# Sindhu-Hegde/jegal

Hardware: AMD Instinct MI355X
Metric: clips/sec (T=150 frames, 270x480) embedding extraction (higher is better)
Workload: dtype f16; 1 GPU; BASELINE configs[1]: synthetic batch=32 gesture-only (GestSync conv + JEGAL gesture encoder), uint8 150x270x480x3 clips resident in HBM, seeded synthetic weights; clips_per_gpu=32, frames=150, precision_mode=5, chunk=32, conv1_zero_tile_skip=True, dual_stream=True, parallelism=clip-sharded x1, no data-path collective

## Files before the change

### jegal_amd/csrc/conv1.hip

```cpp
#include "common.h"

#ifdef JG_CLOCK_STAMPS
__device__ unsigned long long jg_clock_stamps_conv1[2 * 1024];
extern "C" int jg_clock_read_conv1(unsigned long long* out, int n) {
    return hipMemcpyFromSymbol(out, HIP_SYMBOL(jg_clock_stamps_conv1), sizeof(unsigned long long) * (n < 2048 ? n : 2048)) == hipSuccess ? 0 : 1;
}
#endif
#include <cstdio>
#include <cstdlib>
#include <cstring>

struct Conv1Args {
    const uint8_t* src;
    int nclip, T, pad, P;
    const f16* Wd;
    float scale;
    f16* out;
    f16* edge;
    f16* dump;
    int nstrips;
    float invP;
    int zskip;
    const unsigned* zmask;
    const f16* zconst;
    int fill_partial;
};

namespace {
constexpr int IH = 270, IW = 480;
constexpr int PH = 43, PW = 78;
constexpr int TROWS = 16;
constexpr int ROW_PITCH = 3744;
constexpr int TILE_BYTES = TROWS * ROW_PITCH;
__device__ __host__ constexpr int slot_off(int x) { return 32 * x + 16 * (x / 3); }
constexpr int ROW_TILES = 22, COL_TILES = 5;
constexpr int CONV_BYTES = 4 * 8 * 32 * 16;
constexpr int CARRY_BYTES = 8 * 32 * 16;
constexpr int OFF_CONV = 2 * TILE_BYTES;
constexpr int OFF_CARRY = OFF_CONV + 2 * CONV_BYTES;
constexpr int OFF_INIT = OFF_CARRY + 2 * CARRY_BYTES;
constexpr int OFF_LIVE = OFF_INIT + 32;
constexpr int OFF_SKIP = OFF_INIT + 256;
constexpr int MAX_WG_STRIPS = 640;
constexpr int LDS_BYTES = OFF_SKIP + 4 * MAX_WG_STRIPS;
constexpr int MAX_WGS = 1024;
constexpr int DUMP_HALVES_PER_WG = 256 * 8;
}

typedef uint32_t u32x3 __attribute__((ext_vector_type(3)));
struct C1Regs { u32x3 w[2][5]; };

__device__ __forceinline__ f16x8 max8(f16x8 a, f16x8 b) {
    return __builtin_elementwise_max(a, b);
}

__device__ __forceinline__ int conv1_s2_of_mask(unsigned sk) {
    const int L = __builtin_ctz(~sk);
    constexpr int C2_OH = (PH - 5) / 2 + 1;
    const int rs = L >= 2 ? L - 2 : 0;
    return rs < C2_OH ? rs : C2_OH - 1;
}

struct Strips {
    int s_lo, r_hi, GX;
    const unsigned* tab;
    bool use_skip;
    __device__ __forceinline__ bool any() const { return s_lo < r_hi && GX > 0; }
    __device__ __forceinline__ unsigned zero_bands(int k) const {
        return use_skip ? (unsigned)__builtin_amdgcn_readfirstlane((int)tab[k]) : 0u;
    }
};
__device__ __forceinline__ Strips conv1_strips(const Conv1Args& a, const char* smem) {
    const int G32 = (int)gridDim.x;
    const int xcd = blockIdx.x & 7, xidx = blockIdx.x >> 3;
    const int GX = (G32 + 7 - xcd) >> 3;
    const int per = (a.nstrips + 7) >> 3;
    const int r_lo = xcd * per, r_hi = (r_lo + per < a.nstrips) ? r_lo + per : a.nstrips;
    return Strips{r_lo + xidx, r_hi, GX, reinterpret_cast<const unsigned*>(smem + OFF_SKIP), a.zmask != nullptr};
}
__device__ __forceinline__ void strip_split(int strip, int& nf, int& j) {
    nf = (int)((unsigned)strip / 5u);
    j = strip - nf * 5;
}
__device__ __forceinline__ unsigned skip_of(unsigned z) { return z & ((z << 1) | 1u); }
struct Walk {
    int strip, rt;
    int k;
    unsigned skip;
    unsigned z;
    bool done;
};
template <class F>
__device__ __forceinline__ void walk_next(const Strips& S, Walk& q, F&& on_strip) {
    if (q.done) return;
    while (true) {
        if (++q.rt == ROW_TILES) {
            q.rt = 0;
            q.strip += S.GX;
            ++q.k;
            if (q.strip >= S.r_hi) { q.done = true; return; }
            q.z = S.zero_bands(q.k);
            q.skip = skip_of(q.z);
            on_strip(q.strip, q.skip);
        }
        if (!((q.skip >> q.rt) & 1u)) return;
    }
}
template <class F>
__device__ __forceinline__ Walk walk_first(const Strips& S, F&& on_strip) {
    Walk q = {S.s_lo, -1, 0, 0u, 0u, !S.any()};
    if (q.done) return q;
    q.z = S.zero_bands(0);
    q.skip = skip_of(q.z);
    on_strip(q.strip, q.skip);
    walk_next(S, q, on_strip);
    return q;
}

__device__ __forceinline__ bool tile_live(const char* smem, int t) {
    return __builtin_amdgcn_readfirstlane(*reinterpret_cast<const int*>(smem + OFF_LIVE + (t & 1) * 4)) != 0;
}
__device__ __forceinline__ bool tile_is_zero(const char* smem, int t) {
    const int4 fl = *reinterpret_cast<const int4*>(smem + OFF_INIT + (t & 1) * 16);
    return __builtin_amdgcn_readfirstlane(fl.x | fl.y | fl.z | fl.w) == 0;
}

struct Mfma32 {
    static constexpr int NSTEP = 49, NCB = 1;
    static constexpr int DEPTH = 6;
    typedef f32x16 Acc;
    const int chalf, r, h;
    f16x8 wreg[49];
    const char* base;
    __device__ __forceinline__ Mfma32(const f16* Wd, int lane, int chalf_) : chalf(chalf_), r(lane & 31), h(lane >> 5) {
#pragma unroll
        for (int s = 0; s < 49; ++s)
            wreg[s] = *reinterpret_cast<const f16x8*>(Wd + conv1_wd_index(s, chalf * 32 + r, 8 * h));
    }
    __device__ __forceinline__ void set_tile(const char* cur) { base = cur + 112 * r + 16 * h; }
    __device__ __forceinline__ f16x8 frag(int gi) const {
        const int q = gi / 49, s = gi - q * 49;
        const int kh = s / 7, kw = s - kh * 7;
        return *reinterpret_cast<const f16x8*>(base + (6 * q + kh) * ROW_PITCH + 32 * kw + 16 * (kw / 3));
    }
    __device__ __forceinline__ static void zero(Acc& acc) {
#pragma unroll
        for (int x = 0; x < 16; ++x) acc[x] = 0.f;
    }
    __device__ __forceinline__ void step(Acc& acc, int s, int, f16x8 f) const {
        acc = __builtin_amdgcn_mfma_f32_32x32x16_f16(wreg[s], f, acc, 0, 0, 0);
    }
    __device__ __forceinline__ void store(const Acc& acc, char* cbuf, int mb, float scale) const {
#pragma unroll
        for (int g = 0; g < 4; ++g) {
            const f16x4 hv = {(f16)fmaxf(acc[4 * g] * scale, 0.f), (f16)fmaxf(acc[4 * g + 1] * scale, 0.f),
                              (f16)fmaxf(acc[4 * g + 2] * scale, 0.f), (f16)fmaxf(acc[4 * g + 3] * scale, 0.f)};
            *reinterpret_cast<f16x4*>(cbuf + ((mb * 8 + chalf * 4 + g) * 32 + r) * 16 + 8 * h) = hv;
        }
    }
};
struct Mfma16 {
    static constexpr int NSTEP = 25, NCB = 2;
    static constexpr int DEPTH = 4;
    struct Acc { f32x4 v[2][2]; };
    const int chalf, n16, kq, sel, half, colp;
    f16x8 wreg[25][2];
    int lb_row, lb_32, lb_224;
    int st_off;
    const char *p_row, *p_32, *p_224;
    __device__ __forceinline__ static void step_slots(int t, int& kha, int& kwa, int& khb, int& kwb) {
        if (t < 21) { kha = 2 * (t / 7); kwa = t % 7; khb = kha + 1; kwb = kwa; }
        else if (t == 21) { kha = khb = 6; kwa = 1; kwb = 2; }
        else if (t == 22) { kha = khb = 6; kwa = 4; kwb = 5; }
        else if (t == 23) { kha = khb = 6; kwa = 0; kwb = 6; }
        else { kha = khb = 6; kwa = 3; kwb = 4; }
    }
    __device__ __forceinline__ Mfma16(const f16* Wd, int lane, int chalf_)
        : chalf(chalf_), n16(lane & 15), kq(lane >> 4), sel(kq & 1), half(kq >> 1),
          colp((n16 >= 4 && n16 < 12) ? 2 * (n16 - 4) : (n16 < 4 ? 2 * n16 + 1 : 2 * (n16 - 8) + 1)) {
#pragma unroll
        for (int t = 0; t < 25; ++t) {
            int kha, kwa, khb, kwb;
            step_slots(t, kha, kwa, khb, kwb);
            const int sl = sel ? khb * 7 + kwb : kha * 7 + kwa;
#pragma unroll
            for (int ob = 0; ob < 2; ++ob) {
                wreg[t][ob] = *reinterpret_cast<const f16x8*>(Wd + conv1_wd_index(sl, chalf * 32 + ob * 16 + n16, 8 * half));
                if (t == 24 && sel) wreg[t][ob] = f16x8{0, 0, 0, 0, 0, 0, 0, 0};
            }
        }
        const int lb = 112 * colp + 16 * half;
        lb_row = lb + sel * ROW_PITCH; lb_32 = lb + sel * 32; lb_224 = lb + sel * 224;
        st_off = ((chalf * 4 + (kq >> 1)) * 32 + colp) * 16 + 8 * (kq & 1);
    }
    __device__ __forceinline__ void set_tile(const char* cur) {
        p_row = cur + lb_row;
        p_32 = cur + lb_32;
        p_224 = cur + lb_224;
    }
    __device__ __forceinline__ f16x8 frag(int gi) const {
        const int q = gi / 50, st = (gi - q * 50) >> 1, cb = gi & 1;
        int kha, kwa, khb, kwb;
        step_slots(st, kha, kwa, khb, kwb);
        const int off = (6 * q + kha) * ROW_PITCH + 32 * kwa + 16 * (kwa / 3) + 1792 * cb;
        const char* pb = st < 21 ? p_row : (st == 23 ? p_224 : p_32);
        return *reinterpret_cast<const f16x8*>(pb + off);
    }
    __device__ __forceinline__ static void zero(Acc& acc) {
#pragma unroll
        for (int ob = 0; ob < 2; ++ob)
#pragma unroll
            for (int cb = 0; cb < 2; ++cb) acc.v[ob][cb] = f32x4{0.f, 0.f, 0.f, 0.f};
    }
    __device__ __forceinline__ void step(Acc& acc, int st, int cb, f16x8 f) const {
        acc.v[0][cb] = __builtin_amdgcn_mfma_f32_16x16x32_f16(wreg[st][0], f, acc.v[0][cb], 0, 0, 0);
        acc.v[1][cb] = __builtin_amdgcn_mfma_f32_16x16x32_f16(wreg[st][1], f, acc.v[1][cb], 0, 0, 0);
    }
    __device__ __forceinline__ void store(const Acc& acc, char* cbuf, int mb, float scale) const {
#pragma unroll
        for (int ob = 0; ob < 2; ++ob)
#pragma unroll
            for (int cb = 0; cb < 2; ++cb) {
                const f32x4 v = acc.v[ob][cb];
                const f16x4 hv = {(f16)fmaxf(v.x * scale, 0.f), (f16)fmaxf(v.y * scale, 0.f), (f16)fmaxf(v.z * scale, 0.f), (f16)fmaxf(v.w * scale, 0.f)};
                *reinterpret_cast<f16x4*>(cbuf + st_off + ((mb * 8 + ob * 2) * 32 + cb * 16) * 16) = hv;
            }
    }
};

template <class Form>
__device__ __forceinline__ void conv1_mfma_role(const f16* Wd, float scale, char* smem, int lane, int wave) {
    constexpr int NSTEP = Form::NSTEP, NCB = Form::NCB, DEPTH = Form::DEPTH, NFRAG = 2 * NSTEP * NCB;
    const int mb0 = (wave >> 1) & 1;
    Form F(Wd, lane, wave & 1);
#ifdef JG_CLOCK_STAMPS
    const unsigned long long ck0 = __builtin_amdgcn_s_memtime(), rt0 = __builtin_amdgcn_s_memrealtime();
#endif
    for (int t = 0;; ++t) {
        __syncthreads();
        if (!tile_live(smem, t)) break;
        F.set_tile(smem + (t & 1) * TILE_BYTES + 3 * mb0 * ROW_PITCH);
        char* cbuf = smem + OFF_CONV + (t & 1) * CONV_BYTES;
        if (tile_is_zero(smem, t)) {
#pragma unroll
            for (int q = 0; q < 2; ++q) {
                typename Form::Acc acc;
                Form::zero(acc);
#pragma unroll
                for (int st = 0; st < 2; ++st)
#pragma unroll
                    for (int cb = 0; cb < NCB; ++cb) F.step(acc, st, cb, F.frag((q * NSTEP + st) * NCB + cb));
                F.store(acc, cbuf, mb0 + 2 * q, scale);
            }
            continue;
        }
        f16x8 fr[DEPTH];
#pragma unroll
        for (int gi = 0; gi < DEPTH; ++gi) fr[gi] = F.frag(gi);
#pragma unroll
        for (int q = 0; q < 2; ++q) {
            typename Form::Acc acc;
            Form::zero(acc);
#pragma unroll
            for (int st = 0; st < NSTEP; ++st)
#pragma unroll
                for (int cb = 0; cb < NCB; ++cb) {
                    const int gi = (q * NSTEP + st) * NCB + cb;
                    F.step(acc, st, cb, fr[gi % DEPTH]);
                    if (gi + DEPTH < NFRAG) fr[gi % DEPTH] = F.frag(gi + DEPTH);
                    __builtin_amdgcn_sched_barrier(0);
                }
            F.store(acc, cbuf, mb0 + 2 * q, scale);
        }
    }
#ifdef JG_CLOCK_STAMPS
    if (wave == 0 && lane == 0 && blockIdx.x < 1024) {
        jg_clock_stamps_conv1[2 * blockIdx.x] = __builtin_amdgcn_s_memtime() - ck0;
        jg_clock_stamps_conv1[2 * blockIdx.x + 1] = __builtin_amdgcn_s_memrealtime() - rt0;
    }
#endif
}

template <bool M16>
__global__ __launch_bounds__(512, 2) void conv1_direct_kernel(Conv1Args a) {
    extern __shared__ __attribute__((aligned(16))) char smem[];
    const int tid = threadIdx.x, lane = tid & 63;
    const int wave = __builtin_amdgcn_readfirstlane(tid >> 6);
    const Strips S = conv1_strips(a, smem);
    if (!S.any()) return;
    if (S.use_skip) {
        unsigned* tab = reinterpret_cast<unsigned*>(smem + OFF_SKIP);
        for (int k = tid; k < MAX_WG_STRIPS; k += 512) {
            const int strip = S.s_lo + k * S.GX;
            int nf, j;
            strip_split(strip, nf, j);
            tab[k] = strip < S.r_hi ? a.zmask[nf] : 0u;
        }
        __syncthreads();
    }
    if (wave >= 4) {
        const int ltid = tid - 256;
        const int row0 = ltid / 25, g0 = ltid - row0 * 25;
        const int it1 = ltid + 256;
        const bool has1 = it1 < TROWS * 25;
        const int row1 = has1 ? it1 / 25 : 0, g1 = has1 ? it1 - row1 * 25 : 0;

        uint32_t fb0_lo = (uint32_t)(uintptr_t)a.src, fb0_hi = (uint32_t)((uintptr_t)a.src >> 32);
        uint32_t fdelta[5] = {0, 0, 0, 0, 0};
        uint32_t ioff[2] = {0, 0};
        auto decode = [&](int strip, int& nf, int& j, int& b, int& pp) {
            strip_split(strip, nf, j);
            b = (int)((float)nf * a.invP);
            pp = nf - b * a.P;
            if (pp < 0) { --b; pp += a.P; }
            else if (pp >= a.P) { ++b; pp -= a.P; }
        };
        auto strip_setup = [&](int strip) {
            int nf, j, b, p;
            decode(strip, nf, j, b, p);
            int f0 = p - a.pad;
            f0 = f0 < 0 ? 0 : (f0 > a.T - 1 ? a.T - 1 : f0);
            const uintptr_t fb = (uintptr_t)(a.src + (size_t)(b * a.T + f0) * (size_t)(IH * IW * 3));
            fb0_lo = __builtin_amdgcn_readfirstlane((uint32_t)fb);
            fb0_hi = __builtin_amdgcn_readfirstlane((uint32_t)(fb >> 32));
#pragma unroll
            for (int dt = 0; dt < 5; ++dt) {
                int f = p + dt - a.pad;
                f = f < 0 ? 0 : (f > a.T - 1 ? a.T - 1 : f);
                fdelta[dt] = __builtin_amdgcn_readfirstlane((uint32_t)(f - f0) * (uint32_t)(IH * IW * 3));
            }
#pragma unroll
            for (int u = 0; u < 2; ++u) {
                const int row = u ? row1 : row0, g = u ? g1 : g0;
                int px = j * 96 + 4 * g;
                px = px < IW ? px : IW - 4;
// ... 52 lines not shown
                        int hb = 0;
                        if (k1 < 15) {
                            const int b1 = 3 * q + k1 % 3;
                            hi = R.w[u][k1 / 3][b1 >> 2];
                            hb = b1 & 3;
                        }
                        d[m] = __builtin_amdgcn_perm(hi, lo, 0x0c000c00u | ((4u + hb) << 16) | (uint32_t)(b0 & 3));
                    }
                    const int x = 4 * g + q;
                    char* dst = buf + row * ROW_PITCH + slot_off(x);
                    *reinterpret_cast<uint4*>(dst) = uint4{d[0], d[1], d[2], d[3]};
                    *reinterpret_cast<uint4*>(dst + 16) = uint4{d[4], d[5], d[6], d[7]};
                }
            }
        };
        const int pcg = (ltid >> 4) & 7, ppw = ltid & 15;
        f16* const dump = a.dump + ((long)blockIdx.x * 256 + ltid) * 8;
        const f16x8 cz = S.use_skip ? *reinterpret_cast<const f16x8*>(a.zconst + pcg * 8) : f16x8{0, 0, 0, 0, 0, 0, 0, 0};
        const int prow = __builtin_amdgcn_readfirstlane(ltid >> 7);
        const int ccol = ltid & 31, ccg = ltid >> 5;
        const int pthr = (prow * PW + ppw) * 64 + pcg * 8;
        auto pool = [&](int strip, int rt, int t, bool fastz, bool carry_const) {
            int nf, j;
            strip_split(strip, nf, j);
            const char* cbuf = smem + OFF_CONV + (t & 1) * CONV_BYTES;
            const char* cin = smem + OFF_CARRY + ((rt & 1) ^ 1) * CARRY_BYTES;
            char* cout = smem + OFF_CARRY + (rt & 1) * CARRY_BYTES;
            auto at = [&](const char* base, int row, int cg, int col) {
                return *reinterpret_cast<const f16x8*>(base + ((row * 8 + cg) * 32 + col) * 16);
            };
            const int c0 = 2 * ppw, c1 = c0 + 1, c2 = c0 + 2 < 32 ? c0 + 2 : 31;
            f16x8 m, cnext;
            if (fastz) {
                m = at(cbuf, 0, pcg, 0);
                cnext = at(cbuf, 0, ccg, 0);
            } else {
                const f16x8 q2 = at(cbuf, 2, ccg, ccol), q3 = at(cbuf, 3, ccg, ccol);
                cnext = max8(q2, q3);
                if (prow == 0) {
                    const f16x8 a0 = carry_const ? cz : at(cin, 0, pcg, c0), a1 = carry_const ? cz : at(cin, 0, pcg, c1),
                                a2 = carry_const ? cz : at(cin, 0, pcg, c2);
                    const f16x8 b0 = at(cbuf, 0, pcg, c0), b1 = at(cbuf, 0, pcg, c1), b2 = at(cbuf, 0, pcg, c2);
                    m = max8(max8(max8(a0, a1), max8(a2, b0)), max8(b1, b2));
                } else {
                    const f16x8 a0 = at(cbuf, 0, pcg, c0), a1 = at(cbuf, 0, pcg, c1), a2 = at(cbuf, 0, pcg, c2);
                    const f16x8 b0 = at(cbuf, 1, pcg, c0), b1 = at(cbuf, 1, pcg, c1), b2 = at(cbuf, 1, pcg, c2);
                    const f16x8 d0 = at(cbuf, 2, pcg, c0), d1 = at(cbuf, 2, pcg, c1), d2 = at(cbuf, 2, pcg, c2);
                    m = max8(max8(max8(a0, a1), max8(a2, b0)), max8(max8(b1, b2), max8(max8(d0, d1), d2)));
                }
            }
            const int ph = 2 * rt - 1 + prow;
            const int pw = 16 * j + ppw;
            {
                const long ub = ((long)nf * PH + (2 * rt - 1)) * (PW * 64) + j * (16 * 64);
                f16* dst = (ph >= 0 && pw < PW) ? a.out + ub + pthr : dump;
                __builtin_nontemporal_store(m, reinterpret_cast<f16x8*>(dst));
            }
            if (ph >= 0 && j > 0 && ppw == 0) {
                f16x8 e;
                if (fastz) e = m;
                else if (prow == 0) e = max8(carry_const ? cz : at(cin, 0, pcg, 0), at(cbuf, 0, pcg, 0));
                else e = max8(max8(at(cbuf, 0, pcg, 0), at(cbuf, 1, pcg, 0)), at(cbuf, 2, pcg, 0));
                *reinterpret_cast<f16x8*>(a.edge + (((long)nf * PH + ph) * 4 + (j - 1)) * 64 + pcg * 8) = e;
            }
            *reinterpret_cast<f16x8*>(cout + (ccg * 32 + ccol) * 16) = cnext;
        };
        auto fill_skipped = [&](int strip, unsigned skip) {
            if (!skip) return;
            const int fill_lo = a.fill_partial ? 2 * conv1_s2_of_mask(skip) : 0;
            int nf, j;
            strip_split(strip, nf, j);
            const int pw = 16 * j + ppw;
            for (unsigned m = skip; m; m &= m - 1) {
                const int rt = __builtin_ctz(m);
                const int ph = 2 * rt - 1 + prow;
                if (ph >= fill_lo && pw < PW)
                    *reinterpret_cast<f16x8*>(a.out + (((long)nf * PH + ph) * PW + pw) * 64 + pcg * 8) = cz;
                if (ph >= fill_lo && j > 0 && ppw == 0)
                    *reinterpret_cast<f16x8*>(a.edge + (((long)nf * PH + ph) * 4 + (j - 1)) * 64 + pcg * 8) = cz;
            }
        };

        int* live = reinterpret_cast<int*>(smem + OFF_LIVE);
        C1Regs RA, RB;
        struct Hist { int strip, rt; unsigned skip; bool zero; bool done; };
        auto on_strip = [&](int strip, unsigned skip) {
            strip_setup(strip);
            fill_skipped(strip, skip);
        };
        Walk qi = walk_first(S, on_strip);
        auto hist = [](const Walk& q) { return Hist{q.strip, q.rt, q.skip, q.rt >= 0 && ((q.z >> q.rt) & 1u) != 0, q.done}; };
        const Hist none = {0, 0, 0u, false, true};
        Hist hA = none, hB = none, hC = none, hD = none;
        int last_rt = 0;
        auto issue_next = [&](C1Regs& R) {
            hD = hC; hC = hB; hB = hA;
            hA = hist(qi);
            if (!qi.done) last_rt = qi.rt;
            issue(last_rt, R);
            walk_next(S, qi, on_strip);
        };
        if (ltid == 0) { live[0] = qi.done ? 0 : 1; live[1] = 0; }
        const bool any_tile = !qi.done;
        issue_next(RA);
        if (any_tile) {
            wait_frames(RA, 0);
            cvt_write(RA, smem, 0, hA.zero);
        }
        issue_next(RB);
        issue_next(RA);
        bool z1 = false, z2 = false;
        auto pool_step = [&](int tprev) {
            const bool above_skipped = hD.rt > 0 && ((hD.skip >> (hD.rt - 1)) & 1u);
            const bool above_zero = hD.rt == 0 || above_skipped || z2;
            pool(hD.strip, hD.rt, tprev, z1 && above_zero, above_skipped);
        };
        int t = 0;
        while (!hC.done) {
            __syncthreads();
            const bool zc0 = tile_is_zero(smem, t);
            if (ltid == 0) live[(t + 1) & 1] = hB.done ? 0 : 1;
            wait_frames(RB, t >= 2 ? 2 : 1);
            if (!hB.done) cvt_write(RB, smem + ((t + 1) & 1) * TILE_BYTES, (t + 1) & 1, hB.zero);
            if (t > 0) pool_step(t - 1);
            issue_next(RB);
            z2 = z1; z1 = zc0;
            ++t;
            if (hC.done) break;
            __syncthreads();
            const bool zc1 = tile_is_zero(smem, t);
            if (ltid == 0) live[(t + 1) & 1] = hB.done ? 0 : 1;
            wait_frames(RA, t >= 2 ? 2 : 1);
            if (!hB.done) cvt_write(RA, smem + ((t + 1) & 1) * TILE_BYTES, (t + 1) & 1, hB.zero);
            pool_step(t - 1);
            issue_next(RA);
            z2 = z1; z1 = zc1;
            ++t;
        }
        asm volatile("s_waitcnt vmcnt(0)" ::: "memory");
        __syncthreads();
        if (t > 0) pool_step(t - 1);
        return;
    }

    if constexpr (M16) conv1_mfma_role<Mfma16>(a.Wd, a.scale, smem, lane, wave);
    else conv1_mfma_role<Mfma32>(a.Wd, a.scale, smem, lane, wave);
}

__global__ void conv1_edge_fix_kernel(f16* __restrict__ out, const f16* __restrict__ edge, long n) {
    const long idx = blockIdx.x * (long)blockDim.x + threadIdx.x;
    if (idx >= n) return;
    const int cg = idx & 7;
    const int j = (idx >> 3) & 3;
    const long rowi = idx >> 5;
    f16* o = out + (rowi * PW + 16 * j + 15) * 64 + cg * 8;
    const f16x8 e = *reinterpret_cast<const f16x8*>(edge + (rowi * 4 + j) * 64 + cg * 8);
    *reinterpret_cast<f16x8*>(o) = max8(*reinterpret_cast<const f16x8*>(o), e);
}

__device__ __forceinline__ f16 conv1_zero_patch_value(const f16* __restrict__ Wd, float scale, int c) {
    const float hi = (float)Wd[conv1_wd_index(0, c, CONV1_BIAS_LANE)], lo = (float)Wd[conv1_wd_index(1, c, CONV1_BIAS_LANE)];
    const float acc = hi * 5.9604644775390625e-8f + lo * 5.9604644775390625e-8f;
    return (f16)fmaxf(acc * scale, 0.f);
}
__global__ void conv1_zconst_kernel(const f16* __restrict__ Wd, float scale, f16* __restrict__ zconst) {
    if (threadIdx.x < 64) zconst[threadIdx.x] = conv1_zero_patch_value(Wd, scale, threadIdx.x);
}

__global__ __launch_bounds__(256) void conv1_zero_scan_kernel(const uint8_t* __restrict__ src, unsigned* __restrict__ zmask,
                                                              const f16* __restrict__ Wd, float scale, f16* __restrict__ zconst) {
    __shared__ int rowz[IH + 2];
    const int tid = threadIdx.x, lane = tid & 63, wave = tid >> 6;
    const uint8_t* fb = src + (size_t)blockIdx.x * (size_t)(IH * IW * 3);
    for (int r = tid; r < IH; r += 256) {
        const uint4 v = *reinterpret_cast<const uint4*>(fb + (size_t)r * (IW * 3) + ((r * 37) % 90) * 16);
        rowz[r] = (v.x | v.y | v.z | v.w) == 0 ? 1 : 0;
    }
    __syncthreads();
    for (int r = wave; r < IH; r += 4) {
        if (!rowz[r]) continue;
        const uint8_t* row = fb + (size_t)r * (IW * 3);
        typedef unsigned u32x4 __attribute__((ext_vector_type(4)));
        u32x4 v = __builtin_nontemporal_load(reinterpret_cast<const u32x4*>(row + lane * 16));
        unsigned nz = v.x | v.y | v.z | v.w;
        if (lane < 26) {
            v = __builtin_nontemporal_load(reinterpret_cast<const u32x4*>(row + 1024 + lane * 16));
            nz |= v.x | v.y | v.z | v.w;
        }
        if (__builtin_amdgcn_ballot_w64(nz != 0) != 0 && lane == 0) rowz[r] = 0;
    }
    __syncthreads();
    if (wave == 0) {
        bool z = lane < ROW_TILES;
        if (z) {
            for (int r = 12 * lane; r < 12 * lane + TROWS; ++r) z = z && (r >= IH || rowz[r]);
        }
        const unsigned long long m = __builtin_amdgcn_ballot_w64(z);
        if (lane == 0) zmask[blockIdx.x] = (unsigned)m & ((1u << ROW_TILES) - 1u);
    }
    if (blockIdx.x == 0 && tid < 64) zconst[tid] = conv1_zero_patch_value(Wd, scale, tid);
    if (blockIdx.x == 0 && tid == 64) reinterpret_cast<int*>(zconst)[CONV1_ROWSKIP_WORD] = 0x7fffffff;
}

__global__ void conv1_skip_mask_kernel(const unsigned* __restrict__ fz, int nclip, int T, int pad, int P, unsigned* __restrict__ skip,
                                       int* __restrict__ s2, int* __restrict__ rowskip_min) {
    const int nf = blockIdx.x * blockDim.x + threadIdx.x;
    int rs = 0x7fffffff;
    if (nf < nclip * P) {
        const int b = nf / P, p = nf - b * P;
        unsigned z = (1u << ROW_TILES) - 1u;
        for (int dt = 0; dt < 5; ++dt) {
            int f = p + dt - pad;
            f = f < 0 ? 0 : (f > T - 1 ? T - 1 : f);
            z &= fz[b * T + f];
        }
        const unsigned sk = skip_of(z);
        skip[nf] = z;
        rs = conv1_s2_of_mask(sk);
        s2[nf] = rs;
    }
#pragma unroll
    for (int d = 32; d >= 1; d >>= 1) {
        const int o = __shfl_xor(rs, d, 64);
        rs = o < rs ? o : rs;
    }
    if ((threadIdx.x & 63) == 0 && rs != 0x7fffffff) atomicMin(rowskip_min, rs);
}

size_t conv1_zmask_elems(int nclip, int T) { return conv1_scan_view(nullptr, nclip, T, CONV1_SCAN_MAX_PAD).words; }
const int* conv1_s2_counts(const unsigned* zscratch, int nclip, int T, int pad) {
    return conv1_scan_view(const_cast<unsigned*>(zscratch), nclip, T, pad).s2();
}

hipError_t launch_conv1_scan(const uint8_t* src, int nclip, int T, int pad, const f16* Wd, float scale, unsigned* zscratch, hipStream_t s) {
    if (nclip * T <= 0) return hipSuccess;
    const int P = T + 2 * pad - 4;
    const Conv1Scan z = conv1_scan_view(zscratch, nclip, T, pad);
    hipLaunchKernelGGL(conv1_zero_scan_kernel, dim3((unsigned)(nclip * T)), dim3(256), 0, s, src, z.frame_mask(), Wd, scale * 16777216.0f,
                       static_cast<f16*>(z.zconst()));
    hipLaunchKernelGGL(conv1_skip_mask_kernel, dim3((unsigned)((nclip * P + 255) / 256)), dim3(256), 0, s, z.frame_mask(), nclip, T, pad, P,
                       z.pos_mask(), z.s2(), z.rowskip_min());
    return hipGetLastError();
}

hipError_t launch_conv1_zconst(const f16* Wd, float scale, f16* zconst, hipStream_t s) {
    hipLaunchKernelGGL(conv1_zconst_kernel, dim3(1), dim3(64), 0, s, Wd, scale * 16777216.0f, zconst);
    return hipGetLastError();
}

hipError_t launch_conv1_direct(const uint8_t* src, int nclip, int T, int pad, const f16* Wd, float scale,
                               f16* out_pooled, f16* edge, const unsigned* zscratch, bool fill_all, const EngineOpts& o, hipStream_t s) {
    static bool attr_set[64] = {};
    if (o.device < 0 || o.device >= 64) return hipErrorInvalidDevice;
    const int num_cu = o.num_cu;
    if (!attr_set[o.device]) {
        const void* ks[2] = {reinterpret_cast<const void*>(conv1_direct_kernel<false>), reinterpret_cast<const void*>(conv1_direct_kernel<true>)};
        for (const void* kf : ks) {
            hipError_t e = hipFuncSetAttribute(kf, hipFuncAttributeMaxDynamicSharedMemorySize, LDS_BYTES);
            if (e != hipSuccess) return e;
        }
        attr_set[o.device] = true;
    }
    Conv1Args a;
    a.src = src; a.nclip = nclip; a.T = T; a.pad = pad; a.P = T + 2 * pad - 4;
    a.dump = edge + (size_t)nclip * (T + 2 * pad - 4) * PH * 4 * 64;
    a.Wd = Wd; a.scale = scale * 16777216.0f; a.out = out_pooled; a.edge = edge;
    if ((long)nclip * a.P >= (1L << 24)) return hipErrorInvalidValue;
    a.nstrips = nclip * a.P * COL_TILES;
    a.invP = 1.0f / (float)a.P;
    a.zskip = o.conv1_zero_skip ? 1 : 0;
    a.zmask = nullptr;
    a.zconst = nullptr;
    a.fill_partial = 0;
    if (num_cu > MAX_WGS) return hipErrorInvalidValue;
    if (a.zskip && zscratch && nclip * T > 0 && (a.nstrips + num_cu - 1) / num_cu + 8 <= MAX_WG_STRIPS) {
        const Conv1Scan z = conv1_scan_view(const_cast<unsigned*>(zscratch), nclip, T, pad);
        a.zmask = z.pos_mask();
        a.zconst = static_cast<const f16*>(z.zconst());
        if (!fill_all) a.fill_partial = 1;
    }
    if (a.nstrips <= 0) return hipSuccess;
    if (num_cu < 8 && a.nstrips > num_cu) return hipErrorInvalidValue;
    const unsigned grid = (unsigned)(a.nstrips < num_cu ? a.nstrips : num_cu);
    if (o.conv1_mfma16) hipLaunchKernelGGL((conv1_direct_kernel<true>), dim3(grid), dim3(512), LDS_BYTES, s, a);
    else hipLaunchKernelGGL((conv1_direct_kernel<false>), dim3(grid), dim3(512), LDS_BYTES, s, a);
    return hipGetLastError();
}

hipError_t launch_conv1_edge_fix(f16* out_pooled, const f16* edge, long positions, hipStream_t s) {
    const long n = positions * PH * 4 * 8;
    if (n <= 0) return hipSuccess;
    hipLaunchKernelGGL(conv1_edge_fix_kernel, dim3((unsigned)((n + 255) / 256)), dim3(256), 0, s, out_pooled, edge, n);
    return hipGetLastError();
}

size_t conv1_edge_elems(long positions) { return (size_t)positions * PH * 4 * 64 + (size_t)MAX_WGS * DUMP_HALVES_PER_WG; }
```

### jegal_amd/csrc/gemm_plan.hip

```cpp
#include "gemm_plan.h"

#include <algorithm>
#include <cstring>

namespace {

struct Tile { int mi, wm, wn; };

GemmPlan instance(const GemmShape& a, const EngineOpts& o, bool glds, bool w2, Tile t, bool spr = false, int xe = 0, bool c32 = false, bool lnf = false) {
    const int key[10] = {glds, w2, a.conv, t.mi, t.wm, t.wn, lnf, spr, xe, c32};
    GemmPlan p;
    for (int i = 0; i < GEMM_NUM_INSTANCES && p.instance < 0; ++i)
        if (std::equal(key, key + 10, GEMM_INSTANCES[i].key)) p.instance = i;
    if (p.instance < 0) return p;
    p.name = GEMM_INSTANCES[p.instance].name;
    const int bm = (glds ? 16 * t.mi : 64) * t.wm, bn = 64 * t.wn;
    const long tiles = ((a.M + bm - 1) / bm) * ((a.N + bn - 1) / bn);
    p.n_tiles = (a.N + bn - 1) / bn; p.total_tiles = (int)tiles;
    p.lds = glds ? glds_tile(w2, t.mi, t.wm, t.wn).lds() : (size_t)(bm + bn * (w2 ? 2 : 1)) * 128;
    p.grid = (unsigned)tiles;
    if (!glds) return p;
    if ((lnf || o.gemm_persistent) && tiles > o.num_cu) p.grid = (unsigned)o.num_cu;
    const bool pays = tiles > o.num_cu && 2 * (tiles % o.num_cu) < o.num_cu;
    const int auto_stagger = !pays ? 0 : lnf ? (a.K <= 1024 ? 500 : 1400) : (!a.conv && !o.lanes_active ? 300 : 0);
// ... 15 lines not shown
    const long tiles256 = (long)((a.M + 255) / 256) * ((a.N + 127) / 128);
    const long tiles_big = (long)((a.M + 255) / 256) * ((a.N + 255) / 256);
    if (a.conv) {
        const bool after_skip = a.rowmap && a.const_in;
        if (o.gemm_small_tile && (tiles256 < 200 || tiles_big < 224)) return glds(a, o, w2, {2, 4, 2}, after_skip);
        if (!w2 && o.gemm_big_tile && a.N >= 256 && a.N % 256 == 0) return glds(a, o, false, {8, 2, 4}, after_skip);
        if (!w2 && !after_skip && o.gemm_tall_tile && a.N == 128 && a.M >= 512 * 256) return glds(a, o, false, {8, 4, 2});
        return glds(a, o, w2, {4, 4, 2}, after_skip);
    }
    const int nk = (a.K + 63) / 64;
    auto est = [&](int bm, int bn, double kt_us, double epi_us) {
        const long tiles = (long)((a.M + bm - 1) / bm) * ((a.N + bn - 1) / bn);
        return (double)((tiles + o.num_cu - 1) / o.num_cu) * (nk * kt_us + epi_us);
    };
    const bool spr = a.K <= 1024;
    if (a.ln_mode) {
        const int xe = a.ln_mode == 1 ? 1 : 2;
        if (w2) {
            if (est(128, 128, 1.25, 1.0) < est(256, 128, 1.6, 1.6) && o.gemm_tile != 2) return glds(a, o, true, {2, 4, 2}, false, xe);
            return glds(a, o, true, {4, 4, 2}, false, xe);
        }
        const bool big_ok = a.N % 256 == 0;
        if (!big_ok || (est(128, 128, 0.95, 1.0) < est(256, 256, 1.45, 2.7) && o.gemm_tile != 3) || o.gemm_tile == 1)
            return glds(a, o, false, {2, 4, 2}, false, xe);
        return glds(a, o, false, {8, 2, 4}, spr, xe);
    }
    const bool can_big = !w2 && o.gemm_big_tile && a.N >= 256 && a.N % 256 == 0;
    const double e_small = o.gemm_small_tile ? est(128, 128, w2 ? 1.25 : 0.95, 1.0) : 1e30;
    const double e_mid = est(256, 128, w2 ? 1.6 : 1.2, 1.6);
    const double e_big = can_big ? est(256, 256, 1.45, 2.7) : 1e30;
    int pick = e_big <= e_mid && e_big <= e_small ? 3 : (e_mid <= e_small ? 2 : 1);
    if (o.gemm_tile >= 1 && o.gemm_tile <= 3 && (o.gemm_tile != 3 || can_big)) pick = o.gemm_tile;
    if (pick == 1) return glds(a, o, w2, {2, 4, 2});
    if (pick == 3 && !w2) return glds(a, o, false, {8, 2, 4}, spr);
    return glds(a, o, w2, {4, 4, 2});
}

}

GemmPlan plan_gemm(const GemmShape& a, const EngineOpts& o) {
    const GemmPlan rejected;
    if (a.ln_w) {
        if (a.conv || !ln_fusable(a) || (a.bias_clip && (a.rpc < GEMM_LN_CLIP_MIN_RPC || a.nclips <= 0))) return rejected;
        return instance(a, o, true, false, {8, 1, 8}, false, 0, false, true);
    }
    const bool narrow = a.N <= 64;
    if (a.bias_clip) {
        const bool ok = !a.conv && !a.ln_mode && o.gemm_glds && a.rpc >= GEMM_CLIP_MIN_RPC && a.nclips > 0 && a.K % 64 == 0 && a.M >= GEMM_GLDS_MIN_ROWS &&
                        a.lda % 8 == 0 && a.ldw % 8 == 0 && a.N % 128 == 0 && a.out16 && !a.out32 && !a.res && (a.ldc & 7) == 0 && !narrow;
        if (!ok) return rejected;
    }
    if (a.ln_mode) {
        const bool shape_ok = !a.conv && o.gemm_glds && a.K % 64 == 0 && a.M >= GEMM_GLDS_MIN_ROWS && a.lda % 8 == 0 && a.ldw % 8 == 0 && a.N % 128 == 0 &&
                              a.ldc % 8 == 0;
        const bool mode1_ok = a.ln_mode == 1 && a.ln_stats && a.scale && a.bias && a.out16 && !a.out32 && !a.res;
        const bool mode2_ok = a.ln_mode == 2 && a.ln_stats && a.scale && a.bias && a.out16 && a.out_lo && a.xres_hi && a.xres_lo && a.stat_out &&
                              !a.out32 && !a.res && !a.relu;
        if (!shape_ok || !(mode1_ok || mode2_ok) || a.ln_w || a.a_tiled) return rejected;
        return plan_glds(a, o);
    }
    if (a.a_tiled && (a.conv || narrow || !o.gemm_glds || a.K != 512 || a.M < GEMM_GLDS_MIN_ROWS || a.N % 128)) return rejected;
    if (a.conv) {
        if (a.res) return rejected;
        if (a.N % 4 || a.ldc % 4 || a.ldw % 8) return rejected;
        const bool coords_ok = a.H + a.PH < 2048 && a.W + a.PW < 2048 && a.M < ROWMAP_MAX_ROWS;
        if (o.gemm_glds && !a.w2 && a.N == 64 && a.C == 32 && a.K % 32 == 0 && a.K == a.KH * a.KW * 32 && !a.tap_table && !a.rowmap &&
            a.M >= GEMM_GLDS_CONV_MIN_ROWS && coords_ok && a.out16 && !a.out32 && (a.ldc & 7) == 0 && (a.ldw & 7) == 0)
            return glds(a, o, false, {2, 8, 1}, false, 0, true);
        if (narrow) return a.rowmap ? rejected : staged(a, o, 4, 1);
        if (o.gemm_glds && a.M >= GEMM_GLDS_CONV_MIN_ROWS && a.C % 64 == 0 && a.N % 128 == 0 && coords_ok) return plan_glds(a, o);
        if (a.rowmap) return rejected;
        return staged(a, o, 2, 2);
    }
    if (a.N % 4 || a.ldc % 4 || (a.res && a.ldr % 4)) return rejected;
    const bool staged_ok = a.K % 8 == 0 && a.lda % 8 == 0 && a.ldw % 8 == 0;
    if (narrow) return staged_ok ? staged(a, o, 4, 1) : rejected;
    if (o.gemm_glds && a.K % 64 == 0 && a.M >= GEMM_GLDS_MIN_ROWS && a.lda % 8 == 0 && a.ldw % 8 == 0 && a.N % 128 == 0) return plan_glds(a, o);
    return staged_ok ? staged(a, o, 2, 2) : rejected;
}

bool engine_opts_set(EngineOpts& o, const char* name, int value) {
    if (!std::strcmp(name, "conv1_mfma16")) o.conv1_mfma16 = value != 0;
    else if (!std::strcmp(name, "conv1_zero_skip")) o.conv1_zero_skip = value != 0;
    else if (!std::strcmp(name, "attn_mfma")) o.attn_mfma = value != 0;
    else if (!std::strcmp(name, "gemm_glds")) o.gemm_glds = value != 0;
    else if (!std::strcmp(name, "gemm_tall_tile")) o.gemm_tall_tile = value != 0;
    else if (!std::strcmp(name, "gemm_small_tile")) o.gemm_small_tile = value != 0;
    else if (!std::strcmp(name, "gemm_big_tile")) o.gemm_big_tile = value != 0;
    else if (!std::strcmp(name, "gemm_tile")) o.gemm_tile = value;
    else if (!std::strcmp(name, "gemm_counted")) o.gemm_counted = value != 0;
    else if (!std::strcmp(name, "gemm_persistent")) o.gemm_persistent = value != 0;
    else if (!std::strcmp(name, "gemm_stagger")) o.gemm_stagger = value;
    else return false;
    return true;
}

hipError_t engine_opts_init(EngineOpts& o, int device) {
    o.device = device;
    hipDeviceProp_t prop;
    hipError_t e = hipGetDeviceProperties(&prop, device);
    if (e != hipSuccess) return e;
    o.num_cu = prop.multiProcessorCount > 0 ? prop.multiProcessorCount : 256;
    void* z = nullptr;
    e = hipMalloc(&z, 256);
    if (e != hipSuccess) return e;
    e = hipMemset(z, 0, 256);
    if (e != hipSuccess) return e;
    o.zeros = z;
    return hipSuccess;
}

void engine_opts_release(EngineOpts& o) {
    if (o.zeros) (void)hipFree(const_cast<void*>(o.zeros));
    o.zeros = nullptr;
}
```

### jegal_amd/csrc/shared.h

```cpp
#pragma once
#include <hip/hip_runtime.h>
#include <stdint.h>
#include <cstdio>

__host__ __device__ inline int conv_skip_decode(int w, int op) {
    const int s3 = w / 2;
    const int s = op == 0 ? w : s3 - (op - 1);
    return s > 0 ? s : 0;
}
struct ConvRowMap {
    int OH, OW, op;
    int* map;
    int* base;
    int* total;
};

constexpr int X16T_TILE = 65536;
constexpr int X16T_COLBLK = 8192;
constexpr int X16T_ROWBLK = 1024;
constexpr int X16T_QUAD = 256;
__host__ __device__ __forceinline__ constexpr long x16t_row_off(long m) { return (m >> 7) * X16T_TILE + ((m & 127) >> 4) * X16T_ROWBLK + (m & 15) * 16; }
__host__ __device__ __forceinline__ constexpr long x16t_row_off(int m) { return (long)(m >> 7) * X16T_TILE + ((m & 127) >> 4) * X16T_ROWBLK + (m & 15) * 16; }
__host__ __device__ __forceinline__ constexpr long x16t_col_off(int n) { return (long)(n >> 6) * X16T_COLBLK + ((n & 63) >> 4) * X16T_QUAD + (n & 15); }
__host__ __device__ __forceinline__ constexpr long x16t_index(long m, int n) { return x16t_row_off(m) + x16t_col_off(n); }
static_assert(x16t_index(0, 0) == 0 && x16t_index(1, 1) == 17 && x16t_index(16, 16) == 1024 + 256, "x16t: rows of 16 inside a quad, quads, row blocks");
static_assert(x16t_index(128, 64) == 65536 + 8192 && x16t_index(300, 500) == 2 * 65536 + 7 * 8192 + 2 * 1024 + 3 * 256 + 12 * 16 + 4, "x16t: tiles and column blocks");
static_assert(x16t_row_off(300) == x16t_row_off(300L), "x16t: the two widths agree");

constexpr int ROWMAP_ROW_BITS = 24;
constexpr int ROWMAP_MAX_ROWS = 1 << ROWMAP_ROW_BITS;
constexpr int ROWMAP_MAX_S2 = 255;
__host__ __device__ __forceinline__ constexpr int rowmap_entry(int row, int s2) { return row | (s2 << ROWMAP_ROW_BITS); }
__host__ __device__ __forceinline__ constexpr int rowmap_row(int e) { return e & (ROWMAP_MAX_ROWS - 1); }
__host__ __device__ __forceinline__ constexpr int rowmap_s2(int e) { return (int)((unsigned)e >> ROWMAP_ROW_BITS); }
static_assert(rowmap_entry(5, 3) == 0x03000005 && rowmap_row(0x03000005) == 5 && rowmap_s2(0x03000005) == 3, "row map entry");
static_assert(rowmap_row(rowmap_entry(ROWMAP_MAX_ROWS - 1, ROWMAP_MAX_S2)) == 0xffffff && rowmap_s2(rowmap_entry(ROWMAP_MAX_ROWS - 1, ROWMAP_MAX_S2)) == 255,
              "row map entry: both limits survive the sign bit");

__host__ __device__ __forceinline__ constexpr int mfma32_row(int i, int half) { return (i & 3) + 8 * (i >> 2) + 4 * half; }
static_assert(mfma32_row(0, 0) == 0 && mfma32_row(5, 1) == 13 && mfma32_row(15, 1) == 31, "32x32 accumulator rows");

__host__ __device__ __forceinline__ constexpr long ln_part_index(long row, int nblk, int blk) { return 2 * (row * nblk + blk); }
static_assert(ln_part_index(0, 12, 1) == 2 && ln_part_index(3, 12, 5) == 82, "LayerNorm partial sums");

constexpr int CONV1_BIAS_LANE = 15;
__host__ __device__ __forceinline__ constexpr long conv1_wd_index(int slot, int ch, int e) { return (long)(slot * 64 + ch) * 16 + e; }
static_assert(conv1_wd_index(0, 0, CONV1_BIAS_LANE) == 15 && conv1_wd_index(1, 2, 3) == 1059 && conv1_wd_index(48, 63, 15) == 49 * 64 * 16 - 1, "conv1 weight panel");

constexpr int CONV1_ZHDR_WORDS = 64;
constexpr int CONV1_ROWSKIP_WORD = 32;
constexpr int CONV1_SCAN_MAX_PAD = 12;
struct Conv1Scan {
    unsigned* z;
    size_t frame_off, pos_off, s2_off, words;
    void* zconst() const { return z; }
    int* rowskip_min() const { return reinterpret_cast<int*>(z) + CONV1_ROWSKIP_WORD; }
    unsigned* frame_mask() const { return z + frame_off; }
    unsigned* pos_mask() const { return z + pos_off; }
    int* s2() const { return reinterpret_cast<int*>(z + s2_off); }
};
inline Conv1Scan conv1_scan_view(unsigned* zscratch, int nclip, int T, int pad) {
    Conv1Scan v;
    v.z = zscratch;
    v.frame_off = CONV1_ZHDR_WORDS;
    v.pos_off = v.frame_off + (size_t)nclip * T;
    v.s2_off = v.pos_off + (size_t)nclip * (T + 2 * pad - 4);
    v.words = v.s2_off + (size_t)nclip * (T + 2 * pad - 4);
    return v;
}

inline int grid_for(long total) { return (int)((total + 255) / 256 < 65536 * 4 ? (total + 255) / 256 : 65536 * 4); }

enum { LN_STD = 0, LN_ANNOTATED = 1 };

struct EngineOpts {
    int device = 0;
    int num_cu = 256;
    const void* zeros = nullptr;
    bool gemm_glds = true;
    bool gemm_persistent = true;
    bool gemm_big_tile = true, gemm_small_tile = true, gemm_tall_tile = true;
    int gemm_tile = 0;
    int gemm_counted = 1;
    int gemm_stagger = 0;
    bool lanes_active = false;
    bool attn_mfma = true;
    bool conv1_zero_skip = true;
    bool conv1_mfma16 = true;
    char* kname = nullptr;
};
constexpr int KNAME_LEN = 96;
template <class... T>
inline void record_kernel(char* kname, const char* fmt, T... v) {
    if (kname) snprintf(kname, KNAME_LEN, fmt, v...);
}
hipError_t engine_opts_init(EngineOpts& o, int device);
void engine_opts_release(EngineOpts& o);

hipError_t launch_unpack_masked(const uint8_t* packed, const int* row0, const long long* offs, int n_frames, uint8_t* dst, hipStream_t s,
                                long long packed_bytes = -1);
hipError_t launch_mask_resize(const uint8_t* src, int T, int H, int W, const int* mask_y_dev, uint8_t* dst, hipStream_t s,
                              const long long* offs = nullptr, long long src_bytes = 0);
size_t conv1_zmask_elems(int nclip, int T);
const int* conv1_s2_counts(const unsigned* zscratch, int nclip, int T, int pad);
hipError_t launch_conv_rowmaps(const int* s2, int NF, const ConvRowMap* layers, int nlayers, hipStream_t s);
size_t conv1_edge_elems(long positions);
hipError_t launch_transpose_tokens(const float* in, int N, int L, int D, float* out, hipStream_t s);
hipError_t launch_l2norm(const float* in, float* out, int rows, int D, hipStream_t s);
hipError_t launch_xlmr_embed(const int32_t* ids, int B, int L, int D, int pad_id, int vocab, int maxpos, const float* word, const float* pos,
                             const float* type, float* out, hipStream_t s);
hipError_t launch_ln_stats(const float* part, int rows, int P, float* stats, hipStream_t s);
hipError_t launch_mask_i32_f32(const int32_t* in, float* out, long n, hipStream_t s);
hipError_t launch_logmel(const float* wav, int B, int n_samples, const float* mel_basis, float* out, hipStream_t s);
size_t col_sum_scratch_elems(int K);
size_t rc_scratch_elems(int nclips, int K);
inline bool rc_bias_ok(int N, int K, int tiled) { return (K == 512 || K == 2048) && (!tiled || K == 512) && !(N & 31); }
hipError_t launch_ragged_mean(const float* x, const int32_t* offsets, int n, int D, float* out, hipStream_t s);
hipError_t launch_sim_rank(const float* e1, const float* e2, int n_local, int n_total, int row_offset, int D,
                           int32_t* rank, int32_t* ties, hipStream_t s);
hipError_t launch_spot(const float* g, const float* c, const int32_t* goff, const int32_t* coff, const int32_t* target,
                       int n, int D, float temp, int32_t* pred, float* score, hipStream_t s);
size_t attn_matrix_key_elems(int n_clips);
hipError_t launch_attn_matrix(const float* g, const float* c, const int32_t* goff, const int32_t* coff, int n, int D, int max_frames,
                              float temp, int normalize, float* A, const int64_t* aoff, unsigned long long* keys,
                              int32_t* best_frame, float* best_score, hipStream_t s);
hipError_t launch_asd(const float* q, const float* cand, const int32_t* coff, int n, int D, float temp,
                      int32_t* pred2, hipStream_t s);
```

Before: 2619 clips/s.

## Skip MFMA steps over leading all-zero rows in partially zero conv1 tiles

Extends the zero-mask scan to record the first non-zero image row per frame window, packing it into the upper bits of the per-strip scan word. For each conv1 row tile, the count of leading zero rows is passed through LDS to the MFMA waves. When that count reaches a threshold, the waves run a specialised compile-time partial block that skips the kernel-row steps touching only zero input rows. This saves tensor-core work on tiles that straddle the zero/non-zero boundary, at the cost of extra template instantiations, code size, and a new runtime branch.

```diff
diff --git a/jegal_amd/csrc/conv1.hip b/jegal_amd/csrc/conv1.hip
--- a/jegal_amd/csrc/conv1.hip
+++ b/jegal_amd/csrc/conv1.hip
@@ -23,6 +23,7 @@
     int zskip;
     const unsigned* zmask;
     const f16* zconst;
+    int zpart_min;
     int fill_partial;
 };
 
@@ -34,16 +35,19 @@
 constexpr int TILE_BYTES = TROWS * ROW_PITCH;
 __device__ __host__ constexpr int slot_off(int x) { return 32 * x + 16 * (x / 3); }
 constexpr int ROW_TILES = 22, COL_TILES = 5;
+static_assert(ROW_TILES == CONV1_BAND_BITS, "one band bit per row tile below the scan word's row count");
 constexpr int CONV_BYTES = 4 * 8 * 32 * 16;
 constexpr int CARRY_BYTES = 8 * 32 * 16;
 constexpr int OFF_CONV = 2 * TILE_BYTES;
 constexpr int OFF_CARRY = OFF_CONV + 2 * CONV_BYTES;
 constexpr int OFF_INIT = OFF_CARRY + 2 * CARRY_BYTES;
 constexpr int OFF_LIVE = OFF_INIT + 32;
+constexpr int OFF_ZROWS = OFF_LIVE + 8;
 constexpr int OFF_SKIP = OFF_INIT + 256;
 constexpr int MAX_WG_STRIPS = 640;
 constexpr int LDS_BYTES = OFF_SKIP + 4 * MAX_WG_STRIPS;
 constexpr int MAX_WGS = 1024;
+constexpr int CONV1_PARTIAL_MIN_Z = 5;
 constexpr int DUMP_HALVES_PER_WG = 256 * 8;
 }
 
@@ -66,7 +70,7 @@
     const unsigned* tab;
     bool use_skip;
     __device__ __forceinline__ bool any() const { return s_lo < r_hi && GX > 0; }
-    __device__ __forceinline__ unsigned zero_bands(int k) const {
+    __device__ __forceinline__ unsigned scan_word(int k) const {
         return use_skip ? (unsigned)__builtin_amdgcn_readfirstlane((int)tab[k]) : 0u;
     }
 };
@@ -88,7 +92,13 @@
     int k;
     unsigned skip;
     unsigned z;
+    int lead;
     bool done;
+    __device__ __forceinline__ void enter(unsigned word) {
+        z = conv1_scan_bands(word);
+        lead = conv1_scan_lead(word);
+        skip = skip_of(z);
+    }
 };
 template <class F>
 __device__ __forceinline__ void walk_next(const Strips& S, Walk& q, F&& on_strip) {
@@ -99,8 +109,7 @@
             q.strip += S.GX;
             ++q.k;
             if (q.strip >= S.r_hi) { q.done = true; return; }
-            q.z = S.zero_bands(q.k);
-            q.skip = skip_of(q.z);
+            q.enter(S.scan_word(q.k));
             on_strip(q.strip, q.skip);
         }
         if (!((q.skip >> q.rt) & 1u)) return;
@@ -108,10 +117,9 @@
 }
 template <class F>
 __device__ __forceinline__ Walk walk_first(const Strips& S, F&& on_strip) {
-    Walk q = {S.s_lo, -1, 0, 0u, 0u, !S.any()};
+    Walk q = {S.s_lo, -1, 0, 0u, 0u, 0, !S.any()};
     if (q.done) return q;
-    q.z = S.zero_bands(0);
-    q.skip = skip_of(q.z);
+    q.enter(S.scan_word(0));
     on_strip(q.strip, q.skip);
     walk_next(S, q, on_strip);
     return q;
@@ -124,10 +132,14 @@
     const int4 fl = *reinterpret_cast<const int4*>(smem + OFF_INIT + (t & 1) * 16);
     return __builtin_amdgcn_readfirstlane(fl.x | fl.y | fl.z | fl.w) == 0;
 }
+__device__ __forceinline__ int tile_zero_rows(const char* smem, int t) {
+    return __builtin_amdgcn_readfirstlane(*reinterpret_cast<const int*>(smem + OFF_ZROWS + (t & 1) * 4));
+}
 
 struct Mfma32 {
     static constexpr int NSTEP = 49, NCB = 1;
     static constexpr int DEPTH = 6;
+    __device__ __host__ static constexpr int start_step(int nz) { return 7 * nz; }
     typedef f32x16 Acc;
     const int chalf, r, h;
     f16x8 wreg[49];
@@ -175,6 +187,7 @@
         else if (t == 23) { kha = khb = 6; kwa = 0; kwb = 6; }
         else { kha = khb = 6; kwa = 3; kwb = 4; }
     }
+    __device__ __host__ static constexpr int start_step(int nz) { return nz >= 7 ? NSTEP : 7 * (nz / 2); }
     __device__ __forceinline__ Mfma16(const f16* Wd, int lane, int chalf_)
         : chalf(chalf_), n16(lane & 15), kq(lane >> 4), sel(kq & 1), half(kq >> 1),
           colp((n16 >= 4 && n16 < 12) ? 2 * (n16 - 4) : (n16 < 4 ? 2 * n16 + 1 : 2 * (n16 - 8) + 1)) {
@@ -228,8 +241,33 @@
     }
 };
 
+template <class Form, int START>
+__device__ __forceinline__ void conv1_partial_block(const Form& F, typename Form::Acc& acc) {
+    constexpr int NCB = Form::NCB, DEPTH = Form::DEPTH;
+    constexpr int NRUN = START < 2 ? Form::NSTEP : 2 + Form::NSTEP - START;
+    constexpr int NFRAG = NRUN * NCB;
+    auto step_of = [](int i) { return (START < 2 || i < 2) ? i : START + i - 2; };
+    f16x8 fr[DEPTH];
+#pragma unroll
+    for (int k = 0; k < DEPTH; ++k)
+        if (k < NFRAG) fr[k] = F.frag(step_of(k / NCB) * NCB + k % NCB);
+#pragma unroll
+    for (int k = 0; k < NFRAG; ++k) {
+        F.step(acc, step_of(k / NCB), k % NCB, fr[k % DEPTH]);
+        if (k + DEPTH < NFRAG) fr[k % DEPTH] = F.frag(step_of((k + DEPTH) / NCB) * NCB + (k + DEPTH) % NCB);
+        __builtin_amdgcn_sched_barrier(0);
+    }
+}
+template <class Form, int NZ = 0>
+__device__ __forceinline__ void conv1_partial_run(const Form& F, int nz, typename Form::Acc& acc) {
+    if constexpr (NZ == 7) conv1_partial_block<Form, Form::start_step(7)>(F, acc);
+    else if constexpr (Form::start_step(NZ) == Form::start_step(NZ + 1)) conv1_partial_run<Form, NZ + 1>(F, nz, acc);
+    else if (nz <= NZ) conv1_partial_block<Form, Form::start_step(NZ)>(F, acc);
+    else conv1_partial_run<Form, NZ + 1>(F, nz, acc);
+}
+
 template <class Form>
-__device__ __forceinline__ void conv1_mfma_role(const f16* Wd, float scale, char* smem, int lane, int wave) {
+__device__ __forceinline__ void conv1_mfma_role(const f16* Wd, float scale, int zpart_min, char* smem, int lane, int wave) {
     constexpr int NSTEP = Form::NSTEP, NCB = Form::NCB, DEPTH = Form::DEPTH, NFRAG = 2 * NSTEP * NCB;
     const int mb0 = (wave >> 1) & 1;
     Form F(Wd, lane, wave & 1);
@@ -251,6 +289,20 @@
 #pragma unroll
                     for (int cb = 0; cb < NCB; ++cb) F.step(acc, st, cb, F.frag((q * NSTEP + st) * NCB + cb));
                 F.store(acc, cbuf, mb0 + 2 * q, scale);
+            }
+            continue;
+        }
+        const int zrows = tile_zero_rows(smem, t);
+        if (zrows >= zpart_min) {
+#pragma nounroll
+            for (int q = 0; q < 2; ++q) {
+                const int mb = mb0 + 2 * q;
+                const int nz = zrows - 3 * mb < 0 ? 0 : (zrows - 3 * mb > 7 ? 7 : zrows - 3 * mb);
+                F.set_tile(smem + (t & 1) * TILE_BYTES + 3 * mb * ROW_PITCH);
+                typename Form::Acc acc;
+                Form::zero(acc);
+                conv1_partial_run<Form>(F, nz, acc);
+                F.store(acc, cbuf, mb, scale);
             }
             continue;
         }
@@ -469,15 +521,18 @@
         };
 
         int* live = reinterpret_cast<int*>(smem + OFF_LIVE);
+        int* zrows = reinterpret_cast<int*>(smem + OFF_ZROWS);
         C1Regs RA, RB;
-        struct Hist { int strip, rt; unsigned skip; bool zero; bool done; };
+        struct Hist { int strip, rt; unsigned skip; bool zero; int zrows; bool done; };
         auto on_strip = [&](int strip, unsigned skip) {
             strip_setup(strip);
             fill_skipped(strip, skip);
         };
         Walk qi = walk_first(S, on_strip);
-        auto hist = [](const Walk& q) { return Hist{q.strip, q.rt, q.skip, q.rt >= 0 && ((q.z >> q.rt) & 1u) != 0, q.done}; };
-        const Hist none = {0, 0, 0u, false, true};
+        auto hist = [](const Walk& q) {
+            return Hist{q.strip, q.rt, q.skip, q.rt >= 0 && ((q.z >> q.rt) & 1u) != 0, q.rt >= 0 ? conv1_tile_zero_rows(q.lead, q.rt) : 0, q.done};
+        };
+        const Hist none = {0, 0, 0u, false, 0, true};
         Hist hA = none, hB = none, hC = none, hD = none;
         int last_rt = 0;
         auto issue_next = [&](C1Regs& R) {
@@ -487,7 +542,7 @@
             issue(last_rt, R);
             walk_next(S, qi, on_strip);
         };
-        if (ltid == 0) { live[0] = qi.done ? 0 : 1; live[1] = 0; }
+        if (ltid == 0) { live[0] = qi.done ? 0 : 1; live[1] = 0; zrows[0] = hist(qi).zrows; }
         const bool any_tile = !qi.done;
         issue_next(RA);
         if (any_tile) {
@@ -506,7 +561,7 @@
         while (!hC.done) {
             __syncthreads();
             const bool zc0 = tile_is_zero(smem, t);
-            if (ltid == 0) live[(t + 1) & 1] = hB.done ? 0 : 1;
+            if (ltid == 0) { live[(t + 1) & 1] = hB.done ? 0 : 1; zrows[(t + 1) & 1] = hB.zrows; }
             wait_frames(RB, t >= 2 ? 2 : 1);
             if (!hB.done) cvt_write(RB, smem + ((t + 1) & 1) * TILE_BYTES, (t + 1) & 1, hB.zero);
             if (t > 0) pool_step(t - 1);
@@ -516,7 +571,7 @@
             if (hC.done) break;
             __syncthreads();
             const bool zc1 = tile_is_zero(smem, t);
-            if (ltid == 0) live[(t + 1) & 1] = hB.done ? 0 : 1;
+            if (ltid == 0) { live[(t + 1) & 1] = hB.done ? 0 : 1; zrows[(t + 1) & 1] = hB.zrows; }
             wait_frames(RA, t >= 2 ? 2 : 1);
             if (!hB.done) cvt_write(RA, smem + ((t + 1) & 1) * TILE_BYTES, (t + 1) & 1, hB.zero);
             pool_step(t - 1);
@@ -530,8 +585,8 @@
         return;
     }
 
-    if constexpr (M16) conv1_mfma_role<Mfma16>(a.Wd, a.scale, smem, lane, wave);
-    else conv1_mfma_role<Mfma32>(a.Wd, a.scale, smem, lane, wave);
+    if constexpr (M16) conv1_mfma_role<Mfma16>(a.Wd, a.scale, a.zpart_min, smem, lane, wave);
+    else conv1_mfma_role<Mfma32>(a.Wd, a.scale, a.zpart_min, smem, lane, wave);
 }
 
 __global__ void conv1_edge_fix_kernel(f16* __restrict__ out, const f16* __restrict__ edge, long n) {
@@ -583,7 +638,13 @@
             for (int r = 12 * lane; r < 12 * lane + TROWS; ++r) z = z && (r >= IH || rowz[r]);
         }
         const unsigned long long m = __builtin_amdgcn_ballot_w64(z);
-        if (lane == 0) zmask[blockIdx.x] = (unsigned)m & ((1u << ROW_TILES) - 1u);
+        int lead = IH;
+        for (int r0 = 0; r0 < IH && lead == IH; r0 += 64) {
+            const int r = r0 + lane;
+            const unsigned long long nzr = __builtin_amdgcn_ballot_w64(r < IH && !rowz[r]);
+            if (nzr) lead = r0 + __builtin_ctzll(nzr);
+        }
+        if (lane == 0) zmask[blockIdx.x] = conv1_scan_word((unsigned)m & ((1u << ROW_TILES) - 1u), lead);
     }
     if (blockIdx.x == 0 && tid < 64) zconst[tid] = conv1_zero_patch_value(Wd, scale, tid);
     if (blockIdx.x == 0 && tid == 64) reinterpret_cast<int*>(zconst)[CONV1_ROWSKIP_WORD] = 0x7fffffff;
@@ -596,13 +657,16 @@
     if (nf < nclip * P) {
         const int b = nf / P, p = nf - b * P;
         unsigned z = (1u << ROW_TILES) - 1u;
+        int lead = IH;
         for (int dt = 0; dt < 5; ++dt) {
             int f = p + dt - pad;
             f = f < 0 ? 0 : (f > T - 1 ? T - 1 : f);
-            z &= fz[b * T + f];
+            const unsigned w = fz[b * T + f];
+            z &= conv1_scan_bands(w);
+            lead = conv1_scan_lead(w) < lead ? conv1_scan_lead(w) : lead;
         }
         const unsigned sk = skip_of(z);
-        skip[nf] = z;
+        skip[nf] = conv1_scan_word(z, lead);
         rs = conv1_s2_of_mask(sk);
         s2[nf] = rs;
     }
@@ -659,12 +723,14 @@
     a.zmask = nullptr;
     a.zconst = nullptr;
     a.fill_partial = 0;
+    a.zpart_min = TROWS + 1;
     if (num_cu > MAX_WGS) return hipErrorInvalidValue;
     if (a.zskip && zscratch && nclip * T > 0 && (a.nstrips + num_cu - 1) / num_cu + 8 <= MAX_WG_STRIPS) {
         const Conv1Scan z = conv1_scan_view(const_cast<unsigned*>(zscratch), nclip, T, pad);
         a.zmask = z.pos_mask();
         a.zconst = static_cast<const f16*>(z.zconst());
         if (!fill_all) a.fill_partial = 1;
+        if (o.conv1_partial_skip) a.zpart_min = o.conv1_partial_skip == 1 ? CONV1_PARTIAL_MIN_Z : o.conv1_partial_skip;
     }
     if (a.nstrips <= 0) return hipSuccess;
     if (num_cu < 8 && a.nstrips > num_cu) return hipErrorInvalidValue;
diff --git a/jegal_amd/csrc/gemm_plan.hip b/jegal_amd/csrc/gemm_plan.hip
--- a/jegal_amd/csrc/gemm_plan.hip
+++ b/jegal_amd/csrc/gemm_plan.hip
@@ -121,6 +121,7 @@
 bool engine_opts_set(EngineOpts& o, const char* name, int value) {
     if (!std::strcmp(name, "conv1_mfma16")) o.conv1_mfma16 = value != 0;
     else if (!std::strcmp(name, "conv1_zero_skip")) o.conv1_zero_skip = value != 0;
+    else if (!std::strcmp(name, "conv1_partial_skip")) o.conv1_partial_skip = value < 0 ? 0 : (value > 16 ? 16 : value);
     else if (!std::strcmp(name, "attn_mfma")) o.attn_mfma = value != 0;
     else if (!std::strcmp(name, "gemm_glds")) o.gemm_glds = value != 0;
     else if (!std::strcmp(name, "gemm_tall_tile")) o.gemm_tall_tile = value != 0;
diff --git a/jegal_amd/csrc/shared.h b/jegal_amd/csrc/shared.h
--- a/jegal_amd/csrc/shared.h
+++ b/jegal_amd/csrc/shared.h
@@ -47,6 +47,17 @@
 __host__ __device__ __forceinline__ constexpr long conv1_wd_index(int slot, int ch, int e) { return (long)(slot * 64 + ch) * 16 + e; }
 static_assert(conv1_wd_index(0, 0, CONV1_BIAS_LANE) == 15 && conv1_wd_index(1, 2, 3) == 1059 && conv1_wd_index(48, 63, 15) == 49 * 64 * 16 - 1, "conv1 weight panel");
 
+constexpr int CONV1_BAND_BITS = 22;
+__host__ __device__ __forceinline__ constexpr unsigned conv1_scan_word(unsigned bands, int lead) { return bands | ((unsigned)lead << CONV1_BAND_BITS); }
+__host__ __device__ __forceinline__ constexpr unsigned conv1_scan_bands(unsigned w) { return w & ((1u << CONV1_BAND_BITS) - 1u); }
+__host__ __device__ __forceinline__ constexpr int conv1_scan_lead(unsigned w) { return (int)(w >> CONV1_BAND_BITS); }
+static_assert(conv1_scan_word(0x3fffffu, 270) == 0x43bfffffu && conv1_scan_bands(0x43bfffffu) == 0x3fffffu && conv1_scan_lead(0x43bfffffu) == 270 &&
+              conv1_scan_word(0xffu, 110) == 0x1b8000ffu && conv1_scan_lead(0x1b8000ffu) == 110 && conv1_scan_bands(0x1b8000ffu) == 0xffu, "conv1 scan word");
+__host__ __device__ __forceinline__ constexpr int conv1_tile_zero_rows(int lead, int rt) {
+    return lead - 12 * rt < 0 ? 0 : (lead - 12 * rt > 16 ? 16 : lead - 12 * rt);
+}
+static_assert(conv1_tile_zero_rows(110, 8) == 14 && conv1_tile_zero_rows(110, 9) == 2 && conv1_tile_zero_rows(110, 10) == 0 &&
+              conv1_tile_zero_rows(110, 7) == 16 && conv1_tile_zero_rows(270, 21) == 16 && conv1_tile_zero_rows(0, 0) == 0, "zero rows of a conv1 tile");
 constexpr int CONV1_ZHDR_WORDS = 64;
 constexpr int CONV1_ROWSKIP_WORD = 32;
 constexpr int CONV1_SCAN_MAX_PAD = 12;
@@ -86,6 +97,7 @@
     bool lanes_active = false;
     bool attn_mfma = true;
     bool conv1_zero_skip = true;
+    int conv1_partial_skip = 1;
     bool conv1_mfma16 = true;
     char* kname = nullptr;
 };
```

Measured after the change: 2613 clips/s, median of 2. About the same (-0.2%).
